# orm011/mplan2vdl

Measured on AMD Instinct MI355X. Metric: rows/s, TPC-H Q6 SF100 (fused VDL scan), + achieved HBM GB/s in roofline, higher is better.
Workload: dtype int64; 1 GPU; tpch_q6_sf100; rows_total=600037902, rows_per_gpu=600037902, bytes_per_row=28, finalise=local

## Files before the change

mplan2vdl_amd/csrc/vdl_jit.cpp:

```cpp
#include "vdl_jit.h"

#include <dlfcn.h>
#include <fcntl.h>
#include <sys/stat.h>
#include <unistd.h>

#include <atomic>
#include <cerrno>
#include <cstdio>
#include <cstdlib>
#include <cstring>
#include <fstream>
#include <map>
#include <mutex>
#include <sstream>

namespace vdl {
namespace jit {

namespace {

#ifndef VDL_PROJ_U
#define VDL_PROJ_U 4
#endif
// ... 153 lines not shown
    int64_t chi() const { return hi_open ? INT64_MAX : point ? 0 : 1; }
};
RangeShape range_shape(const Domain &dom, int64_t lo, int64_t hi) {
    RangeShape s;
    s.lo_open = lo <= dom.lo;
    s.hi_open = hi >= dom.hi;
    s.point = !s.lo_open && !s.hi_open && lo == hi;
    return s;
}
std::string rt_filter_line(const MsArgs &C, const MScanDesc &D, int c, bool u32) {
    const RangeShape s = range_shape(column_domain(C, c), D.flo[c], D.fhi[c]);
    if (s.lo_open && s.hi_open) return "";
    const std::string v = std::string(u32 ? "(uint32_t)" : "") + "v[" + std::to_string(c) + "][r]";
    const std::string lo = std::string(u32 ? "(uint32_t)" : "") + "Dr.flo[" + std::to_string(c) + "]", hi = std::string(u32 ? "(uint32_t)" : "") + "Dr.fhi[" + std::to_string(c) + "]";
    std::string t = " _Pragma(\"unroll\") for (int r = 0; r < RW; r++) alive[r] = alive[r]";
    if (s.point) t += " & (" + v + " == " + lo + ")";
    else {
        if (!s.lo_open) t += " & (" + v + " >= " + lo + ")";
        if (!s.hi_open) t += " & (" + v + " <= " + hi + ")";
    }
    return t + ";";
}

std::atomic<int64_t> g_compiled{0}, g_from_disk{0}, g_from_memory{0};

}

void counters(int64_t *compiled, int64_t *from_disk, int64_t *from_memory) {
    if (compiled) *compiled = g_compiled.load();
    if (from_disk) *from_disk = g_from_disk.load();
    if (from_memory) *from_memory = g_from_memory.load();
}

static std::string desc_text(Kind kind, const MsArgs &C, const MScanDesc &D, const char *suffix = "", bool rt = false) {
    auto lo_of = [&](int col, int64_t lo, int64_t hi) { return rt ? range_shape(column_domain(C, col), lo, hi).clo() : lo; };
    auto hi_of = [&](int col, int64_t lo, int64_t hi) { return rt ? range_shape(column_domain(C, col), lo, hi).chi() : hi; };
    std::ostringstream o;
    o << "namespace vdl {\n";
    o << "constexpr MsArgs jit_args" << suffix << "() {\n    MsArgs a{};\n";
    o << "    a.ncol = " << C.ncol << "; a.widths = " << C.widths << "ull; a.filtered = " << C.filtered << "u; a.derived = " << C.derived
      << "u; a.lazy = " << C.lazy << "u; a.stages = " << C.stages << "ull; a.queued = " << C.queued << "; a.decode = " << C.decode << "u;\n";
    if (C.packed) o << "    a.packed = " << C.packed << "u; a.pbits = " << C.pbits << "ull;\n";
    if (C.steps) o << "    a.steps = " << C.steps << "u;\n";
    o << "    return a;\n}\n";
    o << "constexpr MScanDesc jit_desc" << suffix << "() {\n    MScanDesc d{};\n";
    o << "    d.nagg = " << D.nagg << "; d.nkey = " << D.nkey << "; d.replicas = " << D.replicas << "; d.pmin = " << lit(D.pmin) << "; d.pcount = " << lit(D.pcount) << ";\n";
// ... 24 lines not shown
        const MAggDesc &a = D.agg[j];
        o << "    d.agg[" << j << "].kind = " << a.kind << "; d.agg[" << j << "].used = " << a.used << "u; d.agg[" << j << "].plain = " << a.plain << "u; d.agg[" << j
          << "].constant = " << lit(a.constant) << ";\n";
        for (int k = 0; k < C.ncol; k++)
            if ((a.used >> k) & 1u) o << "    d.agg[" << j << "].fa[" << k << "] = " << lit(a.fa[k]) << "; d.agg[" << j << "].fs[" << k << "] = " << lit(a.fs[k]) << ";\n";
    }
    if (kind != MSCAN) {
        o << "    d.take = " << D.take << "u; d.nout = " << D.nout << "; d.bitmap_only = " << D.bitmap_only << "; d.carry = " << D.carry << "u;\n";
        for (int k = 0; k < D.nout; k++) o << "    d.out_col[" << k << "] = " << D.out_col[k] << ";\n";
        o << "    d.nexpr = " << D.nexpr << ";\n";
        for (int k = 0; k < D.nexpr; k++) o << "    d.expr_at[" << k << "] = " << D.expr_at[k] << "; d.expr_len[" << k << "] = " << D.expr_len[k] << ";\n";
    }
    o << "    return d;\n}\n}  // namespace vdl\n";
    return o.str();
}

std::string scan_source(Kind kind, const MsArgs &C, const MScanDesc &D, const Shape &sh) {
    std::ostringstream o;
    o << "#define VDL_SPEC_UNROLL _Pragma(\"unroll\")\n";
    const bool rt = sh.rt_bounds;
    if (rt) o << "#define VDL_RT_BOUNDS 1\n";
    if (kind == MSCAN && sh.batch) o << "#define VDL_BATCH " << sh.batch << "\n#define VDL_BATCH_NAGG " << D.nagg << "\n";
    if (kind == MSCAN && sh.census) o << "#define VDL_CENSUS 1\n";
    if (kind == MSCAN && C.packed) o << "#define VDL_PACKED 1\n";
    if (kind == MSCAN && C.lazy && C.packed) {
        auto ulit = [](int64_t x) { return std::to_string((uint64_t)x & 0xffffffffull) + "u"; };
        o << "#define VDL_STAGED_PRE";
        for (int c = 0; c < C.ncol; c++) {
            if (!((C.filtered >> c) & 1u) || ((C.lazy >> c) & 1u)) continue;
            if (rt) o << rt_filter_line(C, D, c, (C.packed >> c) & 1u);
            else if ((C.packed >> c) & 1u)
                o << " _Pragma(\"unroll\") for (int r = 0; r < RW; r++) alive[r] = alive[r] & ((uint32_t)v[" << c << "][r] >= " << ulit(D.flo[c]) << ") & ((uint32_t)v[" << c
                  << "][r] <= " << ulit(D.fhi[c]) << ");";
            else
                o << " _Pragma(\"unroll\") for (int r = 0; r < RW; r++) alive[r] = alive[r] & (v[" << c << "][r] >= " << lit(D.flo[c]) << ") & (v[" << c << "][r] <= "
                  << lit(D.fhi[c]) << ");";
        }
        o << "\n#define VDL_STAGED_POST";
        for (int c = 0; c < C.ncol; c++) {
            if (!((C.lazy >> c) & 1u)) continue;
            const int w = C.width(c);
            o << " { const __amdgpu_buffer_rsrc_t rs_ = buf_rsrc((const char *)Cr.ptr[" << c << "] + tile0 * " << w << ", (uint32_t)(tile_rows * " << w
              << ")); _Pragma(\"unroll\") for (int r = 0; r < RW; r++) {";
            if (sh.census)
                o << " { const uint64_t m_ = __ballot(pass[r]); const uint64_t a_ = (uint64_t)Cr.ptr[" << c << "] + (uint64_t)(rowid[r] - Cr.row0) * " << w << "ull;"
                  << " const int ln_ = (int)(threadIdx.x & 63u); int lo_ = ln_ - (int)((a_ & 127ull) / " << w << "ull); if (lo_ < 0) lo_ = 0;"
                  << " const bool first_ = pass[r] && ((m_ >> lo_) & ((1ull << (ln_ - lo_)) - 1ull)) == 0ull;"
                  << " const uint64_t f_ = __ballot(first_); if (ln_ == 0) census_cnt[" << c << "] += (unsigned long long)__popcll(f_); }";
// ... 85 lines not shown
std::string front_source(const MsArgs &Cs, const MScanDesc &Ds, const MsArgs &Ct, const MScanDesc &Dt, const Shape &sh, int nct) {
    std::ostringstream o;
    o << "#define VDL_SPEC_UNROLL _Pragma(\"unroll\")\n";
    if (sh.rt_bounds) o << "#define VDL_RT_BOUNDS 1\n";
    o << "#define VDL_PROJ_U " << VDL_PROJ_U_HOST << "\n#define VDL_FRONT_BATCH " << VDL_FRONT_BATCH_HOST << "\n" << kEmbedded << "\n" << desc_text(SELECT, Cs, Ds, "_s", sh.rt_bounds) << desc_text(TAKE, Ct, Dt, "_t", sh.rt_bounds);
    const char *b = sh.vec ? "true" : "false";
    o << "extern \"C\" __global__ __launch_bounds__(256) void " << entry_name(FRONT) << "(const vdl::MsArgs Csr, const vdl::MScanDesc *__restrict__ Dsp, const vdl::MsArgs Ctr,\n"
         "        const vdl::MScanDesc *__restrict__ Dtp, const vdl::FrontLook lk) {\n"
         "    constexpr vdl::MsArgs Cs = vdl::jit_args_s();\n"
         "    constexpr vdl::MScanDesc Ds = vdl::jit_desc_s();\n"
         "    constexpr vdl::MsArgs Ct = vdl::jit_args_t();\n"
         "    constexpr vdl::MScanDesc Dt = vdl::jit_desc_t();\n"
         "    vdl::project_front_body<" << sh.nc << ", " << nct << ", vdl::kProjU, " << b << ", " << b << ">(Cs, Csr, Ds, *Dsp, Ct, Ctr, Dt, *Dtp, lk);\n}\n";
    return o.str();
}
const char *entry_name(Kind kind) { return kind == MSCAN ? "vdl_jit_mscan" : kind == SELECT ? "vdl_jit_project_select" : kind == FRONT ? "vdl_jit_project_front" : "vdl_jit_project_take"; }
std::string entry_name(Kind kind, const MsArgs &C, const MScanDesc &D, const Shape &sh) {
    if (kind != MSCAN) return entry_name(kind);
    char tag[16];
    snprintf(tag, sizeof tag, "%06llx", (unsigned long long)(fnv(desc_text(kind, C, D, "", sh.rt_bounds)) & 0xffffffull));
    int eager_filters = 0;
    for (int c = 0; c < C.ncol; c++) eager_filters += ((C.filtered >> c) & 1u) && !((C.derived >> c) & 1u) && C.stage(c) == 0;
    return std::string("vdl_jit_mscan_") + (sh.grouped ? "grouped_" : "") + (C.packed ? "packed_" : "") + "u" + std::to_string(sh.u) + (C.lazy ? "_staged" + std::to_string(eager_filters) + "_" : "_") +
           (sh.census ? "census_" : "") + tag + (sh.batch ? "_batch" + std::to_string(sh.batch) : "") + (sh.rt_bounds ? "_rtb" : "");
}

bool compile(const std::string &src, const std::string &arch, std::vector<char> &code, std::string &log, Origin *origin) {
    if (origin) *origin = COMPILED;
    std::string key = std::to_string(fnv(src)) + "_" + std::to_string(src.size()) + "_" + arch;
    {
        Rtc &r0 = rtc();
        int major = 0, minor = 0;
        if (r0.lib && r0.version && r0.version(&major, &minor) == 0) key += "_rtc" + std::to_string(major) + "." + std::to_string(minor);
    }
    {
        std::lock_guard<std::mutex> g(g_mu);
        auto it = g_code.find(key);
        if (it != g_code.end()) { code = it->second; g_from_memory++; if (origin) *origin = FROM_MEMORY; return true; }
    }
    if (const char *dump = getenv("VDL_JIT_DUMP")) {
        std::ofstream f(std::string(dump) + "/vdl_" + key + ".hip");
        f << src;
    }
    const std::string dir = trusted_cache_dir();
    std::string path;
    if (!dir.empty()) {
        path = dir + "/vdl_" + key + ".vdlco";
// ... 39 lines not shown
```

mplan2vdl_amd/csrc/vdl_jit.h:

```cpp
#pragma once
#include <hip/hip_runtime.h>

#include <memory>
#include <string>
#include <vector>

#include "vdl_scan_desc.h"

namespace vdl {
namespace jit {

struct Shape { int nc = 0, u = 0; bool vec = false, grouped = false, der = false;
               bool census = false;
               bool rt_bounds = false;
               int batch = 0; };

enum Kind : int { MSCAN = 0, SELECT = 1, TAKE = 2, FRONT = 3 };
const char *entry_name(Kind kind);
std::string entry_name(Kind kind, const MsArgs &C, const MScanDesc &D, const Shape &sh);
std::string scan_source(Kind kind, const MsArgs &C, const MScanDesc &D, const Shape &sh);
std::string mscan_source(const MsArgs &C, const MScanDesc &D, const Shape &sh);
std::string front_source(const MsArgs &Cs, const MScanDesc &Ds, const MsArgs &Ct, const MScanDesc &Dt, const Shape &sh, int nct);
enum Origin : int { COMPILED = 0, FROM_DISK = 1, FROM_MEMORY = 2 };
bool compile(const std::string &src, const std::string &arch, std::vector<char> &code, std::string &log, Origin *origin = nullptr);
void counters(int64_t *compiled, int64_t *from_disk, int64_t *from_memory);

struct Kernel {
    hipModule_t mod = nullptr;
    hipFunction_t fn = nullptr;
    ~Kernel();
};
std::shared_ptr<Kernel> load(const std::vector<char> &code, std::string &why, const std::string &entry);

}
}
```

mplan2vdl_amd/csrc/vdl_mscan_body.h:

```cpp
#pragma once
#include "vdl_scan_desc.h"

#ifndef VDL_SPEC_UNROLL
#define VDL_SPEC_UNROLL
#endif

namespace vdl {

typedef long long ll2 __attribute__((ext_vector_type(2)));
typedef int i32x2 __attribute__((ext_vector_type(2)));
typedef short i16x2 __attribute__((ext_vector_type(2)));
typedef char i8x2 __attribute__((ext_vector_type(2)));

template <int N> struct IntTag { static constexpr int value = N; };

namespace {


constexpr int kWave = 64;
constexpr int kMsBlock = 256;
#ifndef VDL_PROJ_U
#define VDL_PROJ_U 4
#endif
constexpr int kProjU = VDL_PROJ_U;
// ... 29 lines not shown
    const int o = (int)(on ? off : kBufOut);
    if (W == 8) {
        const auto x = __builtin_amdgcn_raw_buffer_load_b128(rs, o, 0, 0);
        a = (int64_t)(((uint64_t)x[1] << 32) | x[0]); b = (int64_t)(((uint64_t)x[3] << 32) | x[2]);
    } else if (W == 4) {
        const auto x = __builtin_amdgcn_raw_buffer_load_b64(rs, o, 0, 0);
        a = (int32_t)x[0]; b = (int32_t)x[1];
    } else if (W == 2) {
        const uint32_t x = __builtin_amdgcn_raw_buffer_load_b32(rs, o, 0, 0);
        a = (int16_t)(x & 0xffffu); b = (int16_t)(x >> 16);
    } else {
        const uint32_t x = __builtin_amdgcn_raw_buffer_load_b16(rs, o, 0, 0);
        a = (int8_t)(x & 0xffu); b = (int8_t)(x >> 8);
    }
}
template <int W>
__device__ __forceinline__ int64_t buf_load_one(__amdgpu_buffer_rsrc_t rs, bool on, uint32_t off) {
    const int o = (int)(on ? off : kBufOut);
    if (W == 8) { const auto x = __builtin_amdgcn_raw_buffer_load_b64(rs, o, 0, 0); return (int64_t)(((uint64_t)x[1] << 32) | x[0]); }
    if (W == 4) return (int32_t)__builtin_amdgcn_raw_buffer_load_b32(rs, o, 0, 0);
    if (W == 2) return (int16_t)__builtin_amdgcn_raw_buffer_load_b16(rs, o, 0, 0);
    return (int8_t)__builtin_amdgcn_raw_buffer_load_b8(rs, o, 0, 0);
}
__device__ __forceinline__ uint32_t unpack_bits(const uint32_t (&w)[32], int j, int b) {
    const int o = j * b, k = o >> 5, sh = o & 31;
    if (b >= 32) return w[k & 31];
    if (sh + b <= 32) return __builtin_amdgcn_ubfe(w[k & 31], (unsigned)sh, (unsigned)b);
    return __builtin_amdgcn_ubfe(__builtin_amdgcn_alignbit(w[(k + 1) & 31], w[k & 31], (unsigned)sh), 0u, (unsigned)b);
}
__device__ __forceinline__ int64_t img_decode(int64_t e, int64_t base, int64_t scale) {
    return (int64_t)((uint64_t)base + (uint64_t)scale * (uint64_t)e);
}
__host__ __device__ inline int64_t step_groups_padded(int64_t n) { return (n + kProjTile - 1) / kProjTile * (kProjTile / 64); }
__device__ __forceinline__ const uint32_t *step_anchors(const void *p, int64_t n) { return (const uint32_t *)((const uint64_t *)p + step_groups_padded(n)); }
__device__ __forceinline__ int64_t step_sum(int64_t base, uint32_t anchor, uint64_t masked, int w) {
    if (w <= 4) return (int64_t)(int32_t)((uint32_t)base + anchor + (uint32_t)__popcll(masked));
    return (int64_t)((uint64_t)base + (uint64_t)anchor + (uint64_t)__popcll(masked));
}
__device__ __forceinline__ int64_t step_load(const void *p, int64_t n, int64_t base, int w, int64_t r) {
    return step_sum(base, step_anchors(p, n)[r >> 6], ((const uint64_t *)p)[r >> 6] & (~0ull >> (63 - (int)(r & 63))), w);
}
template <int U>
__device__ __forceinline__ void step_tile(const void *p, int64_t n, int64_t base, int64_t sb, int w, int64_t (&v)[2 * U]) {
    static_assert((kMsBlock * 2) % 64 == 0, "a tile's sub-iterations start whole groups apart");
    constexpr int GU = kMsBlock * 2 / 64;
    const uint64_t *hp = (const uint64_t *)p + (base >> 6);
// ... 579 lines not shown
                } else {
#pragma unroll
                    for (int r = 0; r < RW; r++) atomicMin((long long *)&mytab[off[r] + 1 + j], (long long)t[r]);
                }
            } else {
                int64_t s = r_identity(rk);
                if (rk == R_SUM) {
#pragma unroll
                    for (int r = 0; r < RW; r++) s = (int64_t)((uint64_t)s + (uint64_t)(pass[r] ? t[r] : 0));
                } else if (rk == R_MIN) {
#pragma unroll
                    for (int r = 0; r < RW; r++) s = (pass[r] && t[r] < s) ? t[r] : s;
                } else {
#pragma unroll
                    for (int r = 0; r < RW; r++) s = (pass[r] && t[r] > s) ? t[r] : s;
                }
                int64_t *slot = &lds[(int64_t)j * BS + tid];
                *slot = r_combine(rk, *slot, s);
            }
        }
    };

    const int64_t ntiles = Cr.n / TILE;
#ifdef VDL_PACKED
    if (!GROUPED && !DER && C.packed) {
        static_assert(32 % ROWS == 0, "a lane's 32 values of a stripe split into row slices");
        const int lane = tid & (kWave - 1);
        const int wave = __builtin_amdgcn_readfirstlane(tid / kWave);
        const int64_t nstripes = (Cr.n + 2047) / 2048, wstride = (int64_t)gridDim.x * (BS / kWave);
        for (int64_t s = (int64_t)blockIdx.x * (BS / kWave) + wave; s < nstripes; s += wstride) {
            uint32_t pw[NC][32];
#pragma unroll
            for (int c = 0; c < NC; c++) {
                if ((C.packed >> c) & 1u) {
                    const int b = C.bits(c);
                    const char *p = (const char *)Cr.ptr[c] + ((s * b) * kWave + lane) * 4;
#pragma unroll
                    for (int k = 0; k < 32; k++)
                        if (k < b) pw[c][k] = stream_load<NT, uint32_t>(p + (int64_t)k * (kWave * 4));
                }
            }
            __builtin_amdgcn_sched_barrier(0);
            const int64_t tile0 = s * 2048, tile_rows = Cr.n - tile0 < 2048 ? Cr.n - tile0 : 2048;
#pragma unroll
            for (int j0 = 0; j0 < 32; j0 += ROWS) {
                int64_t v[NC][ROWS], rowid[ROWS];
// ... 484 lines not shown
```

mplan2vdl_amd/csrc/vdl_scan_form.h:

```cpp
#pragma once
#include "vdl_scan_desc.h"

namespace vdl {

struct ScanForm {
    enum Kind { EAGER, STAGED, QUEUE, PACKED } kind = EAGER;
    static constexpr int kAllFilters = kMaxVCols;
    int eager_filters = 0;
    bool every_column = false;
    int u = 0;

    static ScanForm from_code(int code, int u = 0) {
        ScanForm f;
        f.u = u;
        f.kind = code <= 0 ? EAGER : code == 3 ? QUEUE : code >= 5 ? PACKED : STAGED;
        if (f.kind == STAGED) f.eager_filters = code == 4 ? kAllFilters : code;
        f.every_column = code >= 6;
        return f;
    }
    const char *suffix() const {
        return kind == EAGER ? "" : kind == QUEUE ? ",queue" : kind == PACKED ? (every_column ? ",packed" : ",packed,late")
             : eager_filters == kAllFilters ? ",lateall" : eager_filters > 1 ? ",late2" : ",late";
    }
};

}
```

mplan2vdl_amd/csrc/vdl_specialise.cpp:

```cpp
#include "vdl_specialise.h"

namespace vdl {
namespace eng {

void count_build(vdl_plan *p, const std::string &role, jit::Origin from) {
    std::pair<int, int> &b = p->jit_builds[role];
    b.first++;
    b.second += from != jit::COMPILED;
}
std::string builds_text(const vdl_plan *p, const std::string &role) {
    const auto it = p->jit_builds.find(role);
    if (it == p->jit_builds.end()) return "";
    return "from cache: " + std::to_string(it->second.second) + " of " + std::to_string(it->second.first) + " builds of " + role + "; ";
}

static jit::Shape jit_shape(const MScanCols &cols, const ScanLaunch &cfg, const ScanForm &f, bool rt) {
    jit::Shape sh;
    sh.rt_bounds = rt;
    mscan_variant_shape(cfg, &sh.nc, &sh.u, &sh.vec, &sh.grouped, &sh.der);
    sh.nc = cols.ncol;
    for (int k = 0; k < cols.ncol; k++) sh.der |= cols.kind[k] != VC_DIRECT;
    const char *u = getenv(sh.grouped ? "VDL_JIT_GROUP_U" : "VDL_JIT_U");
    if (u && atoi(u) >= 1 && atoi(u) <= 8) sh.u = atoi(u);
    if (f.u > 0) sh.u = f.u;
    else if (f.kind == ScanForm::PACKED) sh.u = getenv("VDL_JIT_U") ? atoi(getenv("VDL_JIT_U")) : 2;
    return sh;
}
static std::string jit_name(const jit::Shape &sh, bool image) {
    return "k_mscan_specialised<" + std::to_string(sh.nc) + "," + std::to_string(sh.u) + "," + (sh.vec ? "vec" : "novec") + "," + (sh.grouped ? "grouped" : "global") +
           (sh.der ? ",derived" : "") + (image ? ",img" : "") + ">";
}
static ScanForm form_asked_for() { return getenv("VDL_JIT_LATE") ? ScanForm::from_code(std::max(1, atoi(getenv("VDL_JIT_LATE")))) : ScanForm{}; }

static const std::vector<ScanColumn> &scan_columns(const vdl_plan *p, size_t s) {
    const size_t ns = p->fused.scans.size();
    return s < ns ? p->fused.scans[s].cols : p->fused.gscans[s - ns].cols;
}
static std::string short_name(const std::string &name) { return name.substr(name.find('.') == std::string::npos ? 0 : name.find('.') + 1); }
static std::string stages_text(const vdl_plan *p, size_t s, const MsArgs &args) {
    const std::vector<ScanColumn> &sc = scan_columns(p, s);
    std::string o;
    for (int k = 0; k < args.ncol && k < (int)sc.size(); k++) {
        const int st = args.stage(k);
        if (!st) continue;
        o += (o.empty() ? "" : " ") + short_name(sc[(size_t)k].name) + "@" + (st == 15 ? std::string("last") : st == 14 ? std::string("lookups") : std::to_string(st));
    }
    return o;
}
// ... 71 lines not shown
        out.desc = &d;
        out.args = mscan_args(cols);
        if (f.kind == ScanForm::EAGER) return true;
        MsArgs &args = out.args;
        args.stages = staged_columns(c, cols, d, grouped, &args.lazy, f.kind == ScanForm::QUEUE ? 1 : f.eager_filters);
        if (!args.lazy) { why = "no column to read late"; return false; }
        if (f.kind == ScanForm::QUEUE) {
            int eager = 0;
            for (int k = 0; k < cols.ncol; k++) {
                if (cols.kind[k] != VC_DIRECT) continue;
                if (!((args.lazy >> k) & 1u)) { eager++; if (!cols.filtered[k]) { why = "a column that is no filter would come with the tile"; return false; } }
            }
            if (eager != 1) { why = "the queue form wants exactly one filter column with the tile"; return false; }
            args.queued = 1;
            args.stages = 0;
        }
        return true;
    }
    if (grouped || s >= p->fused.scans.size()) { why = "the packed form serves global aggregate scans only, not grouped scans"; return false; }
    const ScanPlan &sp = p->fused.scans[s];
    for (const ScanColumn &sc : sp.cols)
        if (sc.kind != VC_DIRECT) { why = "the packed form serves scans over table columns only, not scans with derived columns"; return false; }
    if (!c->images) { why = "column images are off"; return false; }
    if (u != 1 && u != 2 && u != 4 && u != 8 && u != 16) { why = "the packed form takes 1, 2, 4, 8 or 16 row pairs per slice (a lane's 32 values of a stripe split evenly)"; return false; }
    out.own_cols = std::make_shared<MScanCols>();
    out.own_desc = std::make_shared<MScanDesc>();
    MScanCols &pc = *out.own_cols;
    MScanDesc &pd = *out.own_desc;
    int64_t bpr = 0;
    bind_mscan(c, sp, pc, pd, &bpr, p->row_offset, f.every_column ? 2 : 1);
    pd.block_partials = d.block_partials;
    out.cols = &pc;
    out.desc = &pd;
    if (pc.ncol > 10) { why = "the packed form takes at most 10 columns"; return false; }
    if (!pc.packed) { why = f.every_column ? "no column has a packed image the scan may read" : "no filter column has a packed image the scan may read"; return false; }
    out.args = mscan_args(pc);
    if (!f.every_column) {
        MsArgs &args = out.args;
        uint32_t used = 0;
        for (int j = 0; j < pd.nagg; j++) if (pd.agg[j].kind != AGG_FIRST) used |= pd.agg[j].used;
        for (int k = 0; k < pc.ncol; k++)
            if (!((pc.packed >> k) & 1u) && !pc.filtered[k] && ((used >> k) & 1u)) { args.stages |= (uint64_t)15 << (4 * k); args.lazy |= 1u << k; }
        if (!args.lazy) { why = "no column to read late"; return false; }
    }
    return true;
}
// ... 20 lines not shown
    count_build(p, "scan " + std::to_string(s), from);
    if (code.size() > (size_t)96 << 10) { why = "the descriptor did not fold (" + std::to_string(code.size()) + " B of code)"; return false; }
    out.k = jit::load(code, why, jit::entry_name(jit::MSCAN, args, desc, sh));
    if (!out.k) return false;
    int per_cu = 0;
    if (hipModuleOccupancyMaxActiveBlocksPerMultiprocessor(&per_cu, out.k->fn, 256, mscan_lds_bytes(desc, grouped)) != hipSuccess || per_cu < 1) {
        (void)hipGetLastError();
        per_cu = 2;
    }
    if (per_cu > 8) per_cu = 8;
    const int64_t tile = (int64_t)256 * 2 * sh.u;
    int64_t grid = (int64_t)c->num_cus * per_cu;
    const int64_t most = f.kind == ScanForm::PACKED ? (img::stripes(out.b.cols->n) + 3) / 4 : out.b.cols->n / tile;
    if (grid > most) grid = most;
    if (grid < 1) grid = 1;
    out.grid = (int)grid; out.per_cu = per_cu; out.code_bytes = code.size(); out.form = f; out.form.u = sh.u;
    out.name = jit_name(sh, out.b.cols->image != 0);
    out.name.insert(out.name.size() - 1, std::string(f.suffix()) + (sh.rt_bounds ? ",rtb" : ""));
    out.stages = stages_text(p, s, args);
    out.packed = packed_text(p, s, *out.b.cols);
    return true;
}
static std::string form_text(const Specialised &sp) {
    return (sp.packed.empty() ? "" : ", packed: " + sp.packed) + (sp.stages.empty() ? "" : ", read late: " + sp.stages);
}
static void install_form(vdl_plan *p, size_t s, const Specialised &sp) {
    int64_t *parts = p->mdesc[s].block_partials;
    p->mcols[s] = *sp.b.cols;
    p->mdesc[s] = *sp.b.desc;
    p->mdesc[s].block_partials = parts;
    p->mcfg[s].grid = sp.grid;
    p->mjit[s] = sp.k;
    p->mjit_form[s] = sp.form;
}
bool specialise_scan(vdl_ctx *c, vdl_plan *p, size_t s, bool grouped, std::string *kname) {
    Specialised sp;
    std::string why;
    const ScanForm late = form_asked_for();
    std::string why_late;
    if (late.kind != ScanForm::EAGER && !build_specialised(c, p, s, grouped, late, p->mcols[s], p->mdesc[s], sp, why_late) && late.kind == ScanForm::PACKED)
        p->jit_note += "scan " + std::to_string(s) + ": no packed form (" + why_late + "); ";
    if (!sp.k && !build_specialised(c, p, s, grouped, ScanForm{}, p->mcols[s], p->mdesc[s], sp, why)) { p->jit_note += "scan " + std::to_string(s) + ": not specialised (" + why + "); "; return false; }
    install_form(p, s, sp);
    *kname = sp.name;
    p->jit_note += "scan " + std::to_string(s) + ": " + sp.name + ", " + std::to_string(sp.code_bytes) + " B of code, " + std::to_string(sp.per_cu) + " blocks/CU" + form_text(sp) + "; " +
                   builds_text(p, "scan " + std::to_string(s));
    return true;
// ... 20 lines not shown
}

void tune_specialised(vdl_ctx *c, vdl_plan *p, int64_t *dev_words) {
    const size_t ns = p->fused.scans.size(), ng = p->fused.gscans.size();
    TimingEvents ev;
    HIP_CHECK(hipEventCreate(&ev.a));
    HIP_CHECK(hipEventCreate(&ev.b));
    auto median_ms = [&](auto &&launch) { return median_launch_ms(c, ev, launch); };
    for (size_t s = 0; s < ns + ng; s++) {
        if (!p->mjit[s]) continue;
        const bool grouped = s >= ns;
        int64_t *out = dev_words + (grouped ? p->gword_offset[s - ns] : p->word_offset[s]);
        Specialised best;
        float best_ms = 0;
        std::string tried;
        std::vector<std::pair<int, int>> cands = {{2, 0}, {3, 0}, {4, 0}, {6, 0}, {0, 1}, {3, 1}, {2, 1}, {1, 1}, {3, 2}, {2, 2}, {4, 2}, {4, 3}, {3, 3}, {6, 3},
                                                  {2, 4}, {3, 4}, {4, 4}};
        int pin_u = 0, pin_late = -1;
        if (const char *pin = getenv("VDL_JIT_PIN")) {
            if (const char *q = strstr(pin, "u=")) pin_u = atoi(q + 2);
            if (const char *q = strstr(pin, "late=")) pin_late = atoi(q + 5);
            if (pin_u > 0) cands = {{pin_u, std::max(pin_late, 0)}};
        }
        std::vector<std::pair<int, int>> packed_forms = {{2, 5}, {4, 5}, {8, 5}, {16, 5}, {2, 6}, {4, 6}, {8, 6}};
        const char *packed_env = getenv("VDL_JIT_PACKED");
        if (pin_u > 0 || (packed_env && strcmp(packed_env, "0") == 0)) packed_forms.clear();
        else if (packed_env && strcmp(packed_env, "only") == 0) cands.clear();
        if (!packed_forms.empty()) {
            BoundForm b;
            std::string why;
            if (!bind_form(c, p, s, grouped, ScanForm::from_code(5), 2, p->mcols[s], p->mdesc[s], b, why) &&
                !bind_form(c, p, s, grouped, ScanForm::from_code(6), 2, p->mcols[s], p->mdesc[s], b, why)) packed_forms.clear();
        }
        cands.insert(cands.end(), packed_forms.begin(), packed_forms.end());
        const MScanCols *cols = &p->mcols[s];
        const MScanDesc *desc = &p->mdesc[s];
        MScanCols plain_cols;
        std::unique_ptr<MScanDesc> plain_desc;
        if (p->mjit_form[s].kind == ScanForm::PACKED) {
            plain_desc = std::make_unique<MScanDesc>();
            int64_t bpr = 0;
            bind_mscan(c, p->fused.scans[s], plain_cols, *plain_desc, &bpr, p->row_offset);
            plain_desc->block_partials = p->mdesc[s].block_partials;
            cols = &plain_cols;
            desc = plain_desc.get();
        }
        int best_u = 0;
        for (auto &cu : cands) {
            const ScanForm f = ScanForm::from_code(cu.second, cu.first ? cu.first : best_u);
            if (f.u <= 0 || (f.kind != ScanForm::PACKED && (int64_t)256 * 2 * f.u > cols->n)) continue;
            if (f.kind == ScanForm::STAGED && f.eager_filters == 1 && cu.first == best_u) continue;
            Specialised cand;
            std::string why;
            if (!build_specialised(c, p, s, grouped, f, *cols, *desc, cand, why)) continue;
            ScanLaunch cfg = p->mcfg[s];
            cfg.grid = cand.grid;
            HIP_CHECK(hipMemcpyAsync(p->mdev[s]->p, cand.b.desc, sizeof(MScanDesc), hipMemcpyHostToDevice, c->stream));
            const float ms = median_ms([&] { HIP_CHECK(launch_mscan(*cand.b.cols, *cand.b.desc, (const MScanDesc *)p->mdev[s]->p, cfg, grouped, false, out, false, c->stream, cand.k->fn)); });
            tried += " u=" + std::to_string(f.u) + f.suffix() + ":" + std::to_string((int)(ms * 1000)) + "us";
            if (!best.k || ms < best_ms * 0.98f) { best = cand; best_ms = ms; }
            if (f.kind == ScanForm::EAGER && (best_u == 0 || cand.k == best.k)) best_u = f.u;
        }
        if (!best.k) continue;
        if (!grouped && use_kscan(p->fused.scans[s]) && p->block_partials[s] && pin_u <= 0) {
            const float ms = median_ms([&] {
                HIP_CHECK(launch_scan(p->sargs[s], p->scfg[s], c->stream));
                HIP_CHECK(launch_scan_finish(p->sargs[s].block_partials, p->scfg[s].grid, p->sargs[s].nagg, nullptr, p->sargs[s], out, c->stream));
            });
            tried += std::string(" k_scan:") + std::to_string((int)(ms * 1000)) + "us";
            if (ms < best_ms * 0.98f) {
                p->kscan[s] = 1;
                p->mjit[s] = nullptr;
                p->jit_note += "scan " + std::to_string(s) + " tuned:" + tried + " -> " + scan_kernel_name(p->scfg[s]) + "; " + builds_text(p, "scan " + std::to_string(s));
                if ((int)s == p->dominant) p->dominant_kernel = std::string(scan_kernel_name(p->scfg[s])) + "_grid" + std::to_string(p->scfg[s].grid);
                continue;
            }
        }
        install_form(p, s, best);
        p->jit_note += "scan " + std::to_string(s) + " tuned:" + tried + " -> " + best.name + (best.packed.empty() ? "" : " (packed: " + best.packed + ")") +
                       (best.stages.empty() ? "" : " (read late: " + best.stages + ")") + "; " + builds_text(p, "scan " + std::to_string(s));
        if ((int)s == p->dominant)
            p->dominant_kernel = best.name + "_grid" + std::to_string(best.grid) + (grouped ? "_rep" + std::to_string(p->mdesc[s].replicas) : "");
    }
    p->description = describe_plan(p);
}

int64_t scan_bytes_moved(vdl_ctx *c, vdl_plan *p, std::string &detail) {
    if (!p->bound || p->dominant < 0) throw Error(VDL_ERR_ARG, "vdl_plan_scan_traffic: run the (fused) plan first");
    const size_t s = (size_t)p->dominant, ns = p->fused.scans.size();
    const bool grouped = s >= ns;
    const std::vector<ScanColumn> &sc = scan_columns(p, s);
    const bool staged = !(!grouped && p->kscan[s]) && p->mjit[s] && p->mjit_form[s].kind != ScanForm::EAGER;
    int64_t total = 0;
    if (!grouped && p->kscan[s]) {
        const ScanArgs &a = p->sargs[s];
        for (int k = 0; k < a.ncol; k++) { total += a.n * a.width[k]; detail += short_name(sc[(size_t)k].name) + "=" + std::to_string(a.n * a.width[k]) + " "; }
        detail += "(every column read with the tile)";
        return total;
    }
    if (!staged) {
        const MScanCols &cols = p->mcols[s];
        for (int k = 0; k < cols.ncol; k++)
            if (cols.kind[k] == VC_DIRECT) { total += cols.n * cols.width[k]; detail += short_name(sc[(size_t)k].name) + "=" + std::to_string(cols.n * cols.width[k]) + " "; }
        detail += "(every column read with the tile)";
        return total;
// ... 5 lines not shown
        throw Error(VDL_ERR_UNSUPPORTED, std::string("the census build of the ") + (packed_form ? "packed" : "staged") + " scan failed: " + why);
    BufP counts = dev_alloc(c, sizeof(unsigned long long) * kMaxVCols);
    BufP words = dev_alloc(c, sizeof(int64_t) * (size_t)std::max<int64_t>(p->n_words, 1));
    HIP_CHECK(hipMemsetAsync(counts->p, 0, sizeof(unsigned long long) * kMaxVCols, c->stream));
    const MScanCols &cols = *cen.b.cols;
    MScanDesc d = *cen.b.desc;
    d.census = (unsigned long long *)counts->p;
    BufP ddev = dev_alloc(c, sizeof(MScanDesc));
    HIP_CHECK(hipMemcpyAsync(ddev->p, &d, sizeof d, hipMemcpyHostToDevice, c->stream));
    ScanLaunch cfg = p->mcfg[s];
    cfg.grid = cen.grid;
    int64_t *out = (int64_t *)words->p + (grouped ? p->gword_offset[s - ns] : p->word_offset[s]);
    HIP_CHECK(launch_mscan(cols, d, (const MScanDesc *)ddev->p, cfg, grouped, false, out, false, c->stream, cen.k->fn));
    unsigned long long lines[kMaxVCols] = {};
    c->fetch_to_host(counts->p, kMaxVCols, (int64_t *)lines, c->stream);
    for (int k = 0; k < cols.ncol; k++) {
        if (cols.kind[k] != VC_DIRECT) continue;
        const bool packed = (cols.packed >> k) & 1u, late = (cen.b.args.lazy >> k) & 1u;
        const int64_t b = packed ? img::packed_dwords(cols.n, cols.pbits[k]) * 4 : late ? (int64_t)lines[k] * 128 : cols.n * cols.width[k];
        total += b;
        detail += short_name(sc[(size_t)k].name) + "=" + std::to_string(b) + (packed ? "(packed: " + std::to_string(cols.pbits[k]) + " bits) " :
                                                                               late ? "(late: " + std::to_string(lines[k]) + " lines of " + std::to_string((cols.n * cols.width[k] + 127) / 128) + ") " : " ");
    }
    detail += "(census of " + cen.name + (packed_form ? ")" : ", full tiles)");
    return total;
}

void jit_check_scans(vdl_ctx *c, vdl_plan *p) {
    if (!p->fused.ok) throw Error(VDL_ERR_UNSUPPORTED, "the plan has no fused scans: " + p->fused.why_not);
    const FusedPlan &F = p->fused;
    const size_t ns = F.scans.size();
    for (size_t s = 0; s < ns + F.gscans.size(); s++) {
        const bool grouped = s >= ns;
        MScanCols cols;
        auto d = std::make_unique<MScanDesc>();
        int64_t bpr = 0;
        if (grouped) bind_mscan(c, F.gscans[s - ns], cols, *d, &bpr, 0);
        else bind_mscan(c, F.scans[s], cols, *d, &bpr, 0);
        p->image_roles["scan" + std::to_string(s)] = image_text(scan_columns(p, s), cols);
        const ScanLaunch cfg = mscan_launch_config(cols, *d, grouped, c->num_cus);
        if (cfg.variant < 0) throw Error(VDL_ERR_UNSUPPORTED, "no scan kernel variant for this shape");
        const ScanForm late = form_asked_for();
        jit::Shape sh = jit_shape(cols, cfg, late, p->jit_rt_bounds);
        if (getenv("VDL_JIT_CENSUS")) sh.census = true;
        std::vector<char> code;
        std::string log;
        BoundForm b;
        if (!bind_form(c, p, s, grouped, late, sh.u, cols, *d, b, log)) {
            p->jit_note += "scan " + std::to_string(s) + ": not specialised (" + log + "); ";
            continue;
        }
        if (!jit::compile(jit::mscan_source(b.args, *b.desc, sh), c->arch, code, log))
            throw Error(VDL_ERR_UNSUPPORTED, "scan " + std::to_string(s) + " does not build: " + log.substr(0, 2000));
        std::string name = jit_name(sh, b.cols->image != 0);
        if (b.args.packed) name.insert(name.size() - 1, late.suffix());
        if (sh.rt_bounds) name.insert(name.size() - 1, ",rtb");
        p->jit_note += "scan " + std::to_string(s) + ": " + name + (b.args.packed ? " (packed: " + packed_text(p, s, *b.cols) + ")" : "") +
                       (b.args.queued ? " (queue)" : b.args.lazy ? " (late)" : "") + ", " + std::to_string(code.size()) + " B of code; ";
    }
}

std::string batch_alone_reason(const vdl_plan *p) {
    if (!p->use_fusion || !p->fused.ok) return "the plan is not fused";
    if (!p->use_jit) return "specialisation is off";
    const FusedPlan &F = p->fused;
    if (!F.gscans.empty()) return "grouped scans are not batched";
    if (F.scans.size() != 1) return "the plan has " + std::to_string(F.scans.size()) + " scans, a batch shares exactly one";
    if (!F.prelude.empty()) return "scans with lookup tables or semi-join sets are not batched";
    for (const ScanColumn &sc : F.scans[0].cols)
        if (sc.kind != VC_DIRECT) return "scans with derived columns are not batched";
    if (F.scans[0].never) return "its filters can hold for no row: there is nothing to scan";
    return "";
}
int batch_cap(int nagg) { return std::min(kMaxBatch, kMaxBatchWords / (1 + std::max(nagg, 0))); }

static jit::Shape batch_shape(const BatchMember &m, const ScanForm &f, int k) {
    jit::Shape sh = jit_shape(m.cols, m.cfg, f, true);
    sh.grouped = false;
    sh.der = false;
    sh.batch = k;
    return sh;
// ... 169 lines not shown
```

Measured before the change: 1341 billion rows/s.

## Add sieve packed-late scan variant using wave ballot masks and grouped late loads

Adds a new packed+late scan form ('sieve') that evaluates eager filters into per-row-slot wave ballot masks, then issues late column loads only for lanes that pass, batched into groups to bound in-flight loads. Whole-empty row slots skip the late loads and aggregation entirely. The form is added to the autotuner candidate list, so it is used only if it measures faster than the existing packed forms. It costs extra compile/tuning time and more register pressure from the larger per-slice arrays.

```diff
diff --git a/mplan2vdl_amd/csrc/vdl_jit.cpp b/mplan2vdl_amd/csrc/vdl_jit.cpp
--- a/mplan2vdl_amd/csrc/vdl_jit.cpp
+++ b/mplan2vdl_amd/csrc/vdl_jit.cpp
@@ -199,6 +199,7 @@
     return t + ";";
 }
 
+constexpr int kSieveMaxLateLoads = 48;
 std::atomic<int64_t> g_compiled{0}, g_from_disk{0}, g_from_memory{0};
 
 }
@@ -269,8 +270,54 @@
     if (rt) o << "#define VDL_RT_BOUNDS 1\n";
     if (kind == MSCAN && sh.batch) o << "#define VDL_BATCH " << sh.batch << "\n#define VDL_BATCH_NAGG " << D.nagg << "\n";
     if (kind == MSCAN && sh.census) o << "#define VDL_CENSUS 1\n";
-    if (kind == MSCAN && C.packed) o << "#define VDL_PACKED 1\n";
-    if (kind == MSCAN && C.lazy && C.packed) {
+    const bool sieve = kind == MSCAN && sh.sieve && C.lazy && C.packed;
+    if (sieve) o << "#define VDL_SIEVE 1\n";
+    else if (kind == MSCAN && C.packed) o << "#define VDL_PACKED 1\n";
+    if (sieve) {
+        auto ulit = [](int64_t x) { return std::to_string((uint64_t)x & 0xffffffffull) + "u"; };
+        auto is_packed = [&](int c) { return ((C.packed >> c) & 1u) != 0; };
+        auto is_lazy = [&](int c) { return ((C.lazy >> c) & 1u) != 0; };
+        int group = 32;
+        while (group > 1 && group * __builtin_popcount(C.lazy) > kSieveMaxLateLoads) group /= 2;
+        o << "#define VDL_SIEVE_GROUP " << group << "\n";
+        o << "#define VDL_SIEVE_RSRC";
+        for (int c = 0; c < C.ncol; c++)
+            if (!is_packed(c))
+                o << " const __amdgpu_buffer_rsrc_t rs" << c << "_ = buf_rsrc((const char *)Cr.ptr[" << c << "] + tile0 * " << C.width(c) << ", (uint32_t)(tile_rows * "
+                  << C.width(c) << "));";
+        o << "\n#define VDL_SIEVE_EAGER";
+        for (int c = 0; c < C.ncol; c++)
+            if (!is_packed(c) && !is_lazy(c))
+                o << " ve[" << c << "][r] = buf_load_one<" << C.width(c) << ">(rs" << c << "_, true, (uint32_t)(64 * j + lane) * " << C.width(c) << "u);";
+        o << "\n#define VDL_SIEVE_FILTER";
+        for (int c = 0; c < C.ncol; c++) {
+            if (!((C.filtered >> c) & 1u) || is_lazy(c)) continue;
+            const bool u32 = is_packed(c);
+            std::string test;
+            if (rt) {
+                const RangeShape s = range_shape(column_domain(C, c), D.flo[c], D.fhi[c]);
+                const std::string lo = std::string(u32 ? "(uint32_t)" : "") + "Dr.flo[" + std::to_string(c) + "]", hi = std::string(u32 ? "(uint32_t)" : "") + "Dr.fhi[" + std::to_string(c) + "]";
+                if (s.point) test = " & mask_of(x_ == " + lo + ")";
+                else test = (s.lo_open ? "" : " & mask_of(x_ >= " + lo + ")") + (s.hi_open ? "" : " & mask_of(x_ <= " + hi + ")");
+                if (test.empty()) continue;
+            } else if (u32) test = " & mask_of(x_ >= " + ulit(D.flo[c]) + ") & mask_of(x_ <= " + ulit(D.fhi[c]) + ")";
+            else test = " & mask_of(x_ >= " + lit(D.flo[c]) + ") & mask_of(x_ <= " + lit(D.fhi[c]) + ")";
+            if (u32) o << " { const uint32_t x_ = unpack_bits(pw[" << c << "], j, " << C.bits(c) << "); mj = mj" << test << "; }";
+            else o << " { const int64_t x_ = ve[" << c << "][r]; mj = mj" << test << "; }";
+        }
+        o << "\n#define VDL_SIEVE_LATE";
+        for (int c = 0; c < C.ncol; c++) {
+            if (!is_lazy(c)) continue;
+            const int w = C.width(c);
+            if (sh.census)
+                o << " { const uint64_t a_ = (uint64_t)Cr.ptr[" << c << "] + (uint64_t)(tile0 + 64 * j + lane) * " << w << "ull;"
+                  << " int lo_ = lane - (int)((a_ & 127ull) / " << w << "ull); if (lo_ < 0) lo_ = 0;"
+                  << " const bool first_ = on && ((m_ >> lo_) & ((1ull << (lane - lo_)) - 1ull)) == 0ull;"
+                  << " const uint64_t f_ = __ballot(first_); if (lane == 0) census_cnt[" << c << "] += (unsigned long long)__popcll(f_); }";
+            o << " vl[" << c << "][r] = buf_load_one<" << w << ">(rs" << c << "_, on, (uint32_t)(64 * j + lane) * " << w << "u);";
+        }
+        o << "\n";
+    } else if (kind == MSCAN && C.lazy && C.packed) {
         auto ulit = [](int64_t x) { return std::to_string((uint64_t)x & 0xffffffffull) + "u"; };
         o << "#define VDL_STAGED_PRE";
         for (int c = 0; c < C.ncol; c++) {
@@ -402,7 +449,8 @@
     int eager_filters = 0;
     for (int c = 0; c < C.ncol; c++) eager_filters += ((C.filtered >> c) & 1u) && !((C.derived >> c) & 1u) && C.stage(c) == 0;
     return std::string("vdl_jit_mscan_") + (sh.grouped ? "grouped_" : "") + (C.packed ? "packed_" : "") + "u" + std::to_string(sh.u) + (C.lazy ? "_staged" + std::to_string(eager_filters) + "_" : "_") +
-           (sh.census ? "census_" : "") + tag + (sh.batch ? "_batch" + std::to_string(sh.batch) : "") + (sh.rt_bounds ? "_rtb" : "");
+           (sh.census ? "census_" : "") + tag + (sh.batch ? "_batch" + std::to_string(sh.batch) : "") + (sh.rt_bounds ? "_rtb" : "") +
+           (sh.sieve && C.lazy && C.packed ? "_sieve" : "");
 }
 
 bool compile(const std::string &src, const std::string &arch, std::vector<char> &code, std::string &log, Origin *origin) {
diff --git a/mplan2vdl_amd/csrc/vdl_jit.h b/mplan2vdl_amd/csrc/vdl_jit.h
--- a/mplan2vdl_amd/csrc/vdl_jit.h
+++ b/mplan2vdl_amd/csrc/vdl_jit.h
@@ -13,6 +13,7 @@
 struct Shape { int nc = 0, u = 0; bool vec = false, grouped = false, der = false;
                bool census = false;
                bool rt_bounds = false;
+               bool sieve = false;
                int batch = 0; };
 
 enum Kind : int { MSCAN = 0, SELECT = 1, TAKE = 2, FRONT = 3 };
diff --git a/mplan2vdl_amd/csrc/vdl_mscan_body.h b/mplan2vdl_amd/csrc/vdl_mscan_body.h
--- a/mplan2vdl_amd/csrc/vdl_mscan_body.h
+++ b/mplan2vdl_amd/csrc/vdl_mscan_body.h
@@ -75,6 +75,16 @@
     if (W == 2) return (int16_t)__builtin_amdgcn_raw_buffer_load_b16(rs, o, 0, 0);
     return (int8_t)__builtin_amdgcn_raw_buffer_load_b8(rs, o, 0, 0);
 }
+#ifdef VDL_SIEVE
+__device__ __forceinline__ uint64_t mask_of(bool x) { return __builtin_amdgcn_ballot_w64(x); }
+__device__ __forceinline__ bool lane_of(uint64_t m) {
+#if __has_builtin(__builtin_amdgcn_inverse_ballot_w64)
+    return __builtin_amdgcn_inverse_ballot_w64(m);
+#else
+    return (m >> (threadIdx.x & (kWave - 1))) & 1ull;
+#endif
+}
+#endif
 __device__ __forceinline__ uint32_t unpack_bits(const uint32_t (&w)[32], int j, int b) {
     const int o = j * b, k = o >> 5, sh = o & 31;
     if (b >= 32) return w[k & 31];
@@ -700,6 +710,85 @@
     };
 
     const int64_t ntiles = Cr.n / TILE;
+#ifdef VDL_SIEVE
+    if (!GROUPED && !DER && C.packed) {
+        constexpr int J = ROWS, G = J < VDL_SIEVE_GROUP ? J : VDL_SIEVE_GROUP;
+        static_assert(32 % J == 0 && J % G == 0, "a lane's 32 values of a stripe split into slices, a slice into groups of late loads");
+        const int lane = tid & (kWave - 1);
+        const int wave = __builtin_amdgcn_readfirstlane(tid / kWave);
+        const int64_t nstripes = (Cr.n + 2047) / 2048, wstride = (int64_t)gridDim.x * (BS / kWave);
+        int64_t scnt = 0;
+        for (int64_t s = (int64_t)blockIdx.x * (BS / kWave) + wave; s < nstripes; s += wstride) {
+            uint32_t pw[NC][32];
+#pragma unroll
+            for (int c = 0; c < NC; c++) {
+                if ((C.packed >> c) & 1u) {
+                    const int b = C.bits(c);
+                    const char *p = (const char *)Cr.ptr[c] + ((s * b) * kWave + lane) * 4;
+#pragma unroll
+                    for (int k = 0; k < 32; k++)
+                        if (k < b) pw[c][k] = stream_load<NT, uint32_t>(p + (int64_t)k * (kWave * 4));
+                }
+            }
+            __builtin_amdgcn_sched_barrier(0);
+            const int64_t tile0 = s * 2048, tile_rows = Cr.n - tile0 < 2048 ? Cr.n - tile0 : 2048;
+            VDL_SIEVE_RSRC
+            int64_t acc[kMaxGroupAggs];
+            VDL_SPEC_UNROLL
+            for (int a = 0; a < nagg; a++) acc[a] = r_identity(rk_of(D.agg[a].kind));
+#pragma unroll
+            for (int j0 = 0; j0 < 32; j0 += J) {
+                uint64_t m[J];
+                int64_t ve[NC][J], vl[NC][J];
+#pragma unroll
+                for (int r = 0; r < J; r++) { const int j = j0 + r; (void)j; VDL_SIEVE_EAGER }
+#pragma unroll
+                for (int r = 0; r < J; r++) { const int j = j0 + r; (void)j; uint64_t mj = ~0ull; VDL_SIEVE_FILTER m[r] = mj; }
+                if (tile_rows < 2048) {
+#pragma unroll
+                    for (int r = 0; r < J; r++) {
+                        const int left = (int)tile_rows - 64 * (j0 + r);
+                        m[r] &= left >= 64 ? ~0ull : left <= 0 ? 0ull : (1ull << left) - 1ull;
+                    }
+                }
+#pragma unroll
+                for (int r = 0; r < J; r++) scnt += __popcll(m[r]);
+#pragma unroll
+                for (int g0 = 0; g0 < J; g0 += G) {
+#pragma unroll
+                for (int r = g0; r < g0 + G; r++) { const int j = j0 + r; const uint64_t m_ = m[r]; const bool on = lane_of(m_); (void)j; (void)m_; (void)on; VDL_SIEVE_LATE }
+                asm volatile("" ::: "memory");
+#pragma unroll
+                for (int r = g0; r < g0 + G; r++) {
+                    if (m[r] != 0) {
+                        const int j = j0 + r;
+                        const bool on = lane_of(m[r]);
+                        int64_t v1[NC][1], rid[1] = {Cr.row0 + tile0 + 64 * j + lane};
+#pragma unroll
+                        for (int c = 0; c < NC; c++)
+                            v1[c][0] = ((C.packed >> c) & 1u) ? (int64_t)unpack_bits(pw[c], j, C.bits(c)) : c >= C.ncol ? 0 : ((C.lazy >> c) & 1u) ? vl[c][r] : ve[c][r];
+                        VDL_SPEC_UNROLL
+                        for (int a = 0; a < nagg; a++) {
+                            const int rk = rk_of(D.agg[a].kind);
+                            int64_t t[1];
+                            eval_term<NC, 1>(D.agg[a], v1, rid, t);
+                            if (rk == R_SUM) acc[a] = (int64_t)((uint64_t)acc[a] + (uint64_t)(on ? t[0] : 0));
+                            else if (rk == R_MIN) acc[a] = (on && t[0] < acc[a]) ? t[0] : acc[a];
+                            else acc[a] = (on && t[0] > acc[a]) ? t[0] : acc[a];
+                        }
+                    }
+                }
+                }
+            }
+            VDL_SPEC_UNROLL
+            for (int a = 0; a < nagg; a++) {
+                int64_t *slot = &lds[(int64_t)a * BS + tid];
+                *slot = r_combine(rk_of(D.agg[a].kind), *slot, acc[a]);
+            }
+        }
+        cnt = lane == 0 ? scnt : 0;
+    } else
+#endif
 #ifdef VDL_PACKED
     if (!GROUPED && !DER && C.packed) {
         static_assert(32 % ROWS == 0, "a lane's 32 values of a stripe split into row slices");
diff --git a/mplan2vdl_amd/csrc/vdl_scan_form.h b/mplan2vdl_amd/csrc/vdl_scan_form.h
--- a/mplan2vdl_amd/csrc/vdl_scan_form.h
+++ b/mplan2vdl_amd/csrc/vdl_scan_form.h
@@ -8,6 +8,7 @@
     static constexpr int kAllFilters = kMaxVCols;
     int eager_filters = 0;
     bool every_column = false;
+    bool sieve = false;
     int u = 0;
 
     static ScanForm from_code(int code, int u = 0) {
@@ -15,13 +16,16 @@
         f.u = u;
         f.kind = code <= 0 ? EAGER : code == 3 ? QUEUE : code >= 5 ? PACKED : STAGED;
         if (f.kind == STAGED) f.eager_filters = code == 4 ? kAllFilters : code;
-        f.every_column = code >= 6;
+        f.every_column = code == 6;
+        f.sieve = code == 7;
         return f;
     }
     const char *suffix() const {
         return kind == EAGER ? "" : kind == QUEUE ? ",queue" : kind == PACKED ? (every_column ? ",packed" : ",packed,late")
              : eager_filters == kAllFilters ? ",lateall" : eager_filters > 1 ? ",late2" : ",late";
     }
+    const char *tried_suffix() const { return kind == PACKED && sieve ? ",packed,late,sieve" : suffix(); }
+    const char *form_note() const { return kind == PACKED && sieve ? " (sieve)" : ""; }
 };
 
 }
diff --git a/mplan2vdl_amd/csrc/vdl_specialise.cpp b/mplan2vdl_amd/csrc/vdl_specialise.cpp
--- a/mplan2vdl_amd/csrc/vdl_specialise.cpp
+++ b/mplan2vdl_amd/csrc/vdl_specialise.cpp
@@ -23,7 +23,8 @@
     const char *u = getenv(sh.grouped ? "VDL_JIT_GROUP_U" : "VDL_JIT_U");
     if (u && atoi(u) >= 1 && atoi(u) <= 8) sh.u = atoi(u);
     if (f.u > 0) sh.u = f.u;
-    else if (f.kind == ScanForm::PACKED) sh.u = getenv("VDL_JIT_U") ? atoi(getenv("VDL_JIT_U")) : 2;
+    else if (f.kind == ScanForm::PACKED) sh.u = getenv("VDL_JIT_U") ? atoi(getenv("VDL_JIT_U")) : f.sieve ? 8 : 2;
+    sh.sieve = f.kind == ScanForm::PACKED && f.sieve;
     return sh;
 }
 static std::string jit_name(const jit::Shape &sh, bool image) {
@@ -141,6 +142,7 @@
     for (const ScanColumn &sc : sp.cols)
         if (sc.kind != VC_DIRECT) { why = "the packed form serves scans over table columns only, not scans with derived columns"; return false; }
     if (!c->images) { why = "column images are off"; return false; }
+    if (f.sieve && u != 4 && u != 8 && u != 16) { why = "the sieve takes 4, 8 or 16 row pairs per slice"; return false; }
     if (u != 1 && u != 2 && u != 4 && u != 8 && u != 16) { why = "the packed form takes 1, 2, 4, 8 or 16 row pairs per slice (a lane's 32 values of a stripe split evenly)"; return false; }
     out.own_cols = std::make_shared<MScanCols>();
     out.own_desc = std::make_shared<MScanDesc>();
@@ -207,7 +209,7 @@
     return true;
 }
 static std::string form_text(const Specialised &sp) {
-    return (sp.packed.empty() ? "" : ", packed: " + sp.packed) + (sp.stages.empty() ? "" : ", read late: " + sp.stages);
+    return (sp.packed.empty() ? "" : ", packed: " + sp.packed) + (sp.stages.empty() ? "" : ", read late: " + sp.stages) + sp.form.form_note();
 }
 static void install_form(vdl_plan *p, size_t s, const Specialised &sp) {
     int64_t *parts = p->mdesc[s].block_partials;
@@ -274,7 +276,7 @@
             if (const char *q = strstr(pin, "late=")) pin_late = atoi(q + 5);
             if (pin_u > 0) cands = {{pin_u, std::max(pin_late, 0)}};
         }
-        std::vector<std::pair<int, int>> packed_forms = {{2, 5}, {4, 5}, {8, 5}, {16, 5}, {2, 6}, {4, 6}, {8, 6}};
+        std::vector<std::pair<int, int>> packed_forms = {{2, 5}, {4, 5}, {8, 5}, {16, 5}, {4, 7}, {8, 7}, {16, 7}, {2, 6}, {4, 6}, {8, 6}};
         const char *packed_env = getenv("VDL_JIT_PACKED");
         if (pin_u > 0 || (packed_env && strcmp(packed_env, "0") == 0)) packed_forms.clear();
         else if (packed_env && strcmp(packed_env, "only") == 0) cands.clear();
@@ -309,7 +311,7 @@
             cfg.grid = cand.grid;
             HIP_CHECK(hipMemcpyAsync(p->mdev[s]->p, cand.b.desc, sizeof(MScanDesc), hipMemcpyHostToDevice, c->stream));
             const float ms = median_ms([&] { HIP_CHECK(launch_mscan(*cand.b.cols, *cand.b.desc, (const MScanDesc *)p->mdev[s]->p, cfg, grouped, false, out, false, c->stream, cand.k->fn)); });
-            tried += " u=" + std::to_string(f.u) + f.suffix() + ":" + std::to_string((int)(ms * 1000)) + "us";
+            tried += " u=" + std::to_string(f.u) + f.tried_suffix() + ":" + std::to_string((int)(ms * 1000)) + "us";
             if (!best.k || ms < best_ms * 0.98f) { best = cand; best_ms = ms; }
             if (f.kind == ScanForm::EAGER && (best_u == 0 || cand.k == best.k)) best_u = f.u;
         }
@@ -330,9 +332,10 @@
         }
         install_form(p, s, best);
         p->jit_note += "scan " + std::to_string(s) + " tuned:" + tried + " -> " + best.name + (best.packed.empty() ? "" : " (packed: " + best.packed + ")") +
-                       (best.stages.empty() ? "" : " (read late: " + best.stages + ")") + "; " + builds_text(p, "scan " + std::to_string(s));
+                       (best.stages.empty() ? "" : " (read late: " + best.stages + ")") + best.form.form_note() + "; " + builds_text(p, "scan " + std::to_string(s));
         if ((int)s == p->dominant)
-            p->dominant_kernel = best.name + "_grid" + std::to_string(best.grid) + (grouped ? "_rep" + std::to_string(p->mdesc[s].replicas) : "");
+            p->dominant_kernel = best.name + "_grid" + std::to_string(best.grid) + (grouped ? "_rep" + std::to_string(p->mdesc[s].replicas) : "") +
+                                 (best.form.kind == ScanForm::PACKED && best.form.sieve ? "_sieve" : "");
     }
     p->description = describe_plan(p);
 }
@@ -384,7 +387,7 @@
         detail += short_name(sc[(size_t)k].name) + "=" + std::to_string(b) + (packed ? "(packed: " + std::to_string(cols.pbits[k]) + " bits) " :
                                                                                late ? "(late: " + std::to_string(lines[k]) + " lines of " + std::to_string((cols.n * cols.width[k] + 127) / 128) + ") " : " ");
     }
-    detail += "(census of " + cen.name + (packed_form ? ")" : ", full tiles)");
+    detail += "(census of " + cen.name + cen.form.form_note() + (packed_form ? ")" : ", full tiles)");
     return total;
 }
 
@@ -418,7 +421,7 @@
         if (b.args.packed) name.insert(name.size() - 1, late.suffix());
         if (sh.rt_bounds) name.insert(name.size() - 1, ",rtb");
         p->jit_note += "scan " + std::to_string(s) + ": " + name + (b.args.packed ? " (packed: " + packed_text(p, s, *b.cols) + ")" : "") +
-                       (b.args.queued ? " (queue)" : b.args.lazy ? " (late)" : "") + ", " + std::to_string(code.size()) + " B of code; ";
+                       (b.args.queued ? " (queue)" : b.args.lazy ? " (late)" : "") + (b.args.packed ? late.form_note() : "") + ", " + std::to_string(code.size()) + " B of code; ";
     }
 }
 
```

Measured after the change: 1295 billion rows/s. -3.4%, worse.
